# Jason-Hoford/inversus-reinforcement-learning

Measured on NVIDIA B200. Metric: env_steps_per_sec, higher is better.
Workload: dtype u32

## Files before the change

inversus-reinforcement-learning_b200/csrc/inversus_b200.cu:

```cuda
#include "inversus_kernels.cuh"

#include <chrono>
#include <cstdio>
#include <cstdlib>
#include <cstring>
#include <new>
#include <thread>
#include <vector>

using namespace inv;

namespace inv_host {
void expand_f32(const uint32_t *bits, float *dst, int64_t lo, int64_t hi, int nthreads);
int hardware_threads();
bool stage_action_ids(int8_t *dst, const int8_t *src, int64_t n);
bool check_action_ids(const int8_t *src, int64_t n);
}

struct inv_sim {
    inv_config cfg;
    int64_t n;
    uint4 *state;
    void *obs1, *obs2;
    float *extra1, *extra2, *reward;
    uint8_t *done, *info, *dbg;
    int32_t *ep_steps;
    double *ep_return, *reward64;
    uint32_t *status;
    const uint32_t *table;
    int sm_count;
    int64_t launches;
    bool was_reset;
    int8_t *h_a1, *h_a2, *d_a1, *d_a2;
    uint32_t *h_status;
    cudaStream_t host_stream, copy_stream;
    cudaEvent_t ev_last;
    bool ev_last_valid, need_device_sync;
    cudaEvent_t ev_kernel[8], ev_bits[8], ev_t0, ev_t1;
    char *d_small, *h_small;
    size_t small_bytes, off_extra1, off_extra2, off_reward, off_steps, off_return, off_done, off_info;
    int host_threads;
    double dma_frac;
    bool dma_frac_auto;
    uint4 *d_bits[2];
    uint32_t *h_bits[2];
    double last_dma_s, last_expand_s;
    char *d_events;
    int32_t *d_ev_counts;
    int64_t *h_ev_count;
    int64_t ev_guess;
    cudaEvent_t ev_events;
};

static thread_local char g_err[512] = "";

// ... 175 lines not shown
    p.mode = s->cfg.mode;
    p.difficulty = s->cfg.difficulty;
    p.max_steps = s->cfg.max_episode_steps;
    p.auto_reset = (s->cfg.flags & INV_FLAG_AUTO_RESET) ? 1 : 0;
    return p;
}

constexpr int kTileEnvs = 32;
#ifndef INV_BF16_E
#define INV_BF16_E 64
#endif
#ifndef INV_BF16_T
#define INV_BF16_T 128
#endif
#ifndef INV_NARROW_E
#define INV_NARROW_E 128
#endif
#ifndef INV_NARROW_T
#define INV_NARROW_T 128
#endif
#ifndef INV_WIDE_MIN_ENVS
#define INV_WIDE_MIN_ENVS 131072
#endif

template <int OP, int DT, bool P2V, bool INDEXED, int E, int T = kThreads>
cudaError_t launch_one(const Params &p, int sm_count, cudaStream_t st)
{
    (void)sm_count;
    auto kern = inv_kernel<OP, DT, P2V, INDEXED, E, T>;
    constexpr size_t smem = smem_bytes<E, P2V, INDEXED, DT>();
    static bool configured[64] = {};
    int dev = 0;
    cudaGetDevice(&dev);
    if (dev < 0 || dev >= 64 || !configured[dev]) {
        cudaError_t e = cudaFuncSetAttribute(kern, cudaFuncAttributeMaxDynamicSharedMemorySize, (int)smem);
        if (e != cudaSuccess) return e;
        if (dev >= 0 && dev < 64) configured[dev] = true;
    }
    const int64_t ntiles = (p.count + E - 1) / E;
    if (ntiles <= 0) return cudaSuccess;
    const unsigned grid = (unsigned)(ntiles < (int64_t)0x7FFFFFFF ? ntiles : (int64_t)0x7FFFFFFF);
    kern<<<grid, T, smem, st>>>(p);
    return cudaGetLastError();
}

template <int OP, int DT, bool P2V, bool INDEXED>
cudaError_t launch_e(const Params &p, int sm_count, cudaStream_t st)
{
    if constexpr (DT == INV_OBS_NONE && !INDEXED && OP != OP_DEBUG) {
        return launch_one<OP, DT, P2V, false, 128, 128>(p, sm_count, st);
    } else if constexpr (OP == OP_STEP && !INDEXED && DT != INV_OBS_F32) {
        constexpr int E = (DT == INV_OBS_BF16 && !P2V) ? INV_BF16_E : INV_NARROW_E;
        constexpr int T = (DT == INV_OBS_BF16 && !P2V) ? INV_BF16_T : INV_NARROW_T;
        return launch_one<OP_STEP, DT, P2V, false, E, T>(p, sm_count, st);
    } else if constexpr (DT == INV_OBS_F32 && !INDEXED && OP != OP_DEBUG) {
        if (p.count >= INV_WIDE_MIN_ENVS) {
            if constexpr (OP == OP_STEP && !P2V) return launch_one<OP, DT, P2V, false, 64, 256>(p, sm_count, st);
            else if constexpr (OP == OP_STEP) return launch_one<OP, DT, P2V, false, 64, 384>(p, sm_count, st);
            else return launch_one<OP, DT, P2V, false, 128, 512>(p, sm_count, st);
        }
        return launch_one<OP, DT, P2V, INDEXED, kTileEnvs>(p, sm_count, st);
    } else {
        return launch_one<OP, DT, P2V, INDEXED, kTileEnvs>(p, sm_count, st);
    }
}

template <int OP, bool INDEXED>
cudaError_t launch(const Params &p, int dt, bool p2v, int sm_count, cudaStream_t st)
{
#define INV_CASE(DTV)                                                                   \
    case DTV:                                                                           \
        return p2v ? launch_e<OP, DTV, true, INDEXED>(p, sm_count, st)                  \
                   : launch_e<OP, DTV, false, INDEXED>(p, sm_count, st);
// ... 90 lines not shown
        return fail(INV_ERR_INVALID_ARG, "Unknown opponent_type");
    if (cfg->difficulty != INV_DIFFICULTY_EASY && cfg->difficulty != INV_DIFFICULTY_HARD)
        return fail(INV_ERR_INVALID_ARG, "inv_create: difficulty must be easy(0) or hard(1)");
    if (cfg->obs_dtype < INV_OBS_F32 || cfg->obs_dtype > INV_OBS_NONE)
        return fail(INV_ERR_INVALID_ARG, "inv_create: unknown obs_dtype");
    if (cfg->max_episode_steps <= 0) return fail(INV_ERR_INVALID_ARG, "inv_create: max_episode_steps must be positive");
    if (cfg->env_id_base < 0 || cfg->env_id_base + cfg->n_envs > 0xFFFFFFFFll)
        return fail(INV_ERR_INVALID_ARG, "inv_create: global env ids must fit 32 bits");
    int ndev = inv_device_count();
    if (ndev <= 0) return fail(INV_ERR_NO_DEVICE, "no CUDA device: this simulator has no CPU fallback");
    if (cfg->device < 0 || cfg->device >= ndev) return fail(INV_ERR_INVALID_ARG, "inv_create: bad device ordinal");
    DeviceGuard g(cfg->device);
    cudaDeviceProp prop;
    CUDA_TRY(cudaGetDeviceProperties(&prop, cfg->device));
    if (prop.major != 10)
        return fail(INV_ERR_NO_DEVICE, "device is not sm_100 (B200): kernels are built for sm_100a only");

    inv_sim *s = new (std::nothrow) inv_sim();
    if (!s) return fail(INV_ERR_INVALID_ARG, "out of host memory");
    memset(s, 0, sizeof(*s));
    s->cfg = *cfg;
    if (cfg->mode == INV_MODE_SELFPLAY) s->cfg.flags |= INV_FLAG_P2_VIEW;
    s->n = cfg->n_envs;
    s->sm_count = prop.multiProcessorCount;
    s->host_threads = inv_host::hardware_threads() > 32 ? 32 : inv_host::hardware_threads();
    s->dma_frac = 0.35;
    s->dma_frac_auto = true;
    const int64_t n = s->n;
    const bool p2v = (s->cfg.flags & INV_FLAG_P2_VIEW) != 0;
    const size_t obs_bytes = (size_t)n * INV_OBS_ELEMS * obs_elem_bytes(cfg->obs_dtype);
#define ALLOC(ptr, bytes)                                                        \
    do {                                                                         \
        cudaError_t e_ = cudaMalloc((void **)&(ptr), (bytes));                   \
        if (e_ != cudaSuccess) {                                                 \
            fail(INV_ERR_CUDA, "cudaMalloc(%s): %s", #ptr, cudaGetErrorString(e_)); \
            inv_destroy(s);                                                      \
            return INV_ERR_CUDA;                                                 \
        }                                                                        \
    } while (0)
    ALLOC(s->state, (size_t)n * INV_PACKED_STATE_BYTES);
    if (obs_bytes) {
        ALLOC(s->obs1, obs_bytes);
        if (p2v) ALLOC(s->obs2, obs_bytes);
    }
    {
        auto up = [](size_t v) { return (v + 255) & ~(size_t)255; };
// ... 83 lines not shown
}

int inv_get_config(const inv_sim *s, inv_config *out)
{
    if (!s || !out) return fail(INV_ERR_INVALID_ARG, "inv_get_config: null argument");
    *out = s->cfg;
    return INV_OK;
}

static void note_launch(inv_sim *s, cudaStream_t st)
{
    s->launches += 1;
    if (st == s->host_stream) return;
    cudaStreamCaptureStatus cap = cudaStreamCaptureStatusNone;
    if (cudaStreamIsCapturing(st, &cap) != cudaSuccess || cap != cudaStreamCaptureStatusNone ||
        cudaEventRecord(s->ev_last, st) != cudaSuccess) {
        cudaGetLastError();
        s->need_device_sync = true;
        return;
    }
    s->ev_last_valid = true;
}

static int order_host_stream(inv_sim *s)
{
    if (s->need_device_sync) CUDA_TRY(cudaDeviceSynchronize());
    else if (s->ev_last_valid) CUDA_TRY(cudaStreamWaitEvent(s->host_stream, s->ev_last, 0));
    return INV_OK;
}

static Params chunk_params(const Params &b, int64_t first, int64_t count, size_t env_bytes)
{
    Params p = b;
    p.state = b.state + first;
    p.count = count;
    if (b.a1) p.a1 = b.a1 + first;
    if (b.a2) p.a2 = b.a2 + first;
    if (b.table) p.table = b.table + first * INV_TABLE_STRIDE;
    p.obs1 = static_cast<char *>(b.obs1) + (size_t)first * env_bytes;
    if (b.obs2) p.obs2 = static_cast<char *>(b.obs2) + (size_t)first * env_bytes;
    if (b.bits1) p.bits1 = b.bits1 + first * 16;
    if (b.bits2) p.bits2 = b.bits2 + first * 16;
    p.extra1 = b.extra1 + first * 4;
    if (b.extra2) p.extra2 = b.extra2 + first * 4;
    p.reward = b.reward + first;
    if (b.reward64) p.reward64 = b.reward64 + first;
    p.done = b.done + first;
    p.info = b.info + first;
    p.dbg = b.dbg + first;
    p.ep_steps = b.ep_steps + first;
    p.ep_return = b.ep_return + first;
    p.env_id_base = b.env_id_base + (uint32_t)first;
    return p;
}

int inv_reset(inv_sim *s, void *stream)
{
    if (!s) return fail(INV_ERR_INVALID_ARG, "inv_reset: null handle");
    DeviceGuard g(s->cfg.device);
    Params p = base_params(s);
    CUDA_TRY((launch<OP_RESET, false>(p, s->cfg.obs_dtype, (s->cfg.flags & INV_FLAG_P2_VIEW) != 0, s->sm_count,
                                      (cudaStream_t)stream)));
    note_launch(s, (cudaStream_t)stream);
    s->was_reset = true;
    return INV_OK;
}

int inv_reset_envs(inv_sim *s, const int64_t *idx_dev, int64_t count, void *stream)
{
    if (!s || (!idx_dev && count > 0)) return fail(INV_ERR_INVALID_ARG, "inv_reset_envs: null argument");
    if (count < 0 || count > s->n) return fail(INV_ERR_INVALID_ARG, "inv_reset_envs: bad count");
    if (count == 0) return INV_OK;
    DeviceGuard g(s->cfg.device);
    Params p = base_params(s);
    p.idx = idx_dev;
    p.count = count;
    CUDA_TRY((launch<OP_RESET, true>(p, s->cfg.obs_dtype, (s->cfg.flags & INV_FLAG_P2_VIEW) != 0, s->sm_count,
                                     (cudaStream_t)stream)));
    note_launch(s, (cudaStream_t)stream);
    return INV_OK;
}

static int step_impl(inv_sim *s, const int8_t *a1, const int8_t *a2, void *stream, uint4 *bits1, uint4 *bits2,
                     int64_t first, int64_t count)
{
    if (!s || !a1) return fail(INV_ERR_INVALID_ARG, "inv_step: null argument");
    if (!s->was_reset) return fail(INV_ERR_NOT_RESET, "inv_step before inv_reset");
    if (s->cfg.mode == INV_MODE_SELFPLAY && !a2)
        return fail(INV_ERR_INVALID_ARG, "opponent_policy required for selfplay mode");
    DeviceGuard g(s->cfg.device);
    Params p = base_params(s);
    p.a1 = a1;
    p.a2 = a2;
    p.bits1 = bits1;
    p.bits2 = bits2;
    if (first != 0 || count != s->n) p = chunk_params(p, first, count, obs_env_bytes(s->cfg.obs_dtype));
    CUDA_TRY((launch<OP_STEP, false>(p, s->cfg.obs_dtype, (s->cfg.flags & INV_FLAG_P2_VIEW) != 0, s->sm_count,
                                     (cudaStream_t)stream)));
    note_launch(s, (cudaStream_t)stream);
    return INV_OK;
}

int inv_step(inv_sim *s, const int8_t *a1, const int8_t *a2, void *stream)
{
    return step_impl(s, a1, a2, stream, nullptr, nullptr, 0, s ? s->n : 0);
}

constexpr int kMaxHostChunks = 8;
constexpr int64_t kHostChunkMinEnvs = 131072;
constexpr size_t kStagedSmallMax = 8u << 20;

struct SmallOut {
    float *extra_p1, *extra_p2, *reward;
    uint8_t *done, *info;
    int32_t *episode_steps;
    double *episode_return;
};

static int ensure_host_staging(inv_sim *s)
{
    const size_t n = (size_t)s->n;
    if (!s->h_a1) CUDA_TRY(cudaMallocHost((void **)&s->h_a1, n));
    if (!s->h_a2) CUDA_TRY(cudaMallocHost((void **)&s->h_a2, n));
    size_t staged_max = kStagedSmallMax;
    if (const char *e = getenv("INV_HOST_STAGED_MAX")) staged_max = (size_t)atoll(e);
    if (!s->h_small && s->small_bytes <= staged_max) CUDA_TRY(cudaMallocHost((void **)&s->h_small, s->small_bytes));
    return INV_OK;
}
// ... 99 lines not shown
                  double *episode_return)
{
    if (!s) return fail(INV_ERR_INVALID_ARG, "inv_step_host: null argument");
    if (obs_p1 && !s->obs1) return fail(INV_ERR_INVALID_ARG, "this handle keeps no observation tensor (INV_OBS_NONE)");
    if (obs_p2 && !s->obs2) return fail(INV_ERR_INVALID_ARG, "P2 view was not enabled (INV_FLAG_P2_VIEW)");
    if (extra_p2 && !s->extra2) return fail(INV_ERR_INVALID_ARG, "P2 view was not enabled (INV_FLAG_P2_VIEW)");
    DeviceGuard g(s->cfg.device);
    int rc = begin_host_step(s, a1, a2, "inv_step_host");
    if (rc != INV_OK) return rc;
    const int64_t n = s->n;
    const bool selfplay = s->cfg.mode == INV_MODE_SELFPLAY;
    const bool expand = use_host_expand(s, obs_p1, obs_p2);
    if (expand && (rc = ensure_bits_staging(s, obs_p2 != nullptr)) != INV_OK) return rc;
    cudaStream_t ks = s->host_stream, cs = s->copy_stream;
    int64_t bounds[kMaxHostChunks + 1];
    const int nchunks = host_chunk_bounds(n, obs_p1 || obs_p2, s->h_small != nullptr, bounds);
    const SmallOut so = {extra_p1, extra_p2, reward, done, info, episode_steps, episode_return};
    const size_t env_bytes = (size_t)INV_OBS_ELEMS * obs_elem_bytes(s->cfg.obs_dtype);
    void *dst[2] = {obs_p1, obs_p2};
    const void *src[2] = {s->obs1, s->obs2};
    const double frac = expand ? s->dma_frac : 1.0;
    int64_t lo[kMaxHostChunks], mid[kMaxHostChunks], hi[kMaxHostChunks];

    int used = 0;
    for (int c = 0; c < nchunks; ++c) {
        const int64_t first = bounds[c];
        if (first >= n) break;
        const int64_t count = bounds[c + 1] - first;
        if (count <= 0) break;
        lo[c] = first;
        hi[c] = first + count;
        mid[c] = expand ? first + ((int64_t)((double)count * frac) & ~(int64_t)255) : first + count;
        rc = step_impl(s, s->d_a1, selfplay ? s->d_a2 : nullptr, ks, expand ? s->d_bits[0] : nullptr,
                       expand && obs_p2 ? s->d_bits[1] : nullptr, first, count);
        if (rc != INV_OK) return rc;
        CUDA_TRY(cudaEventRecord(s->ev_kernel[c], ks));
        used = c + 1;
    }
    CUDA_TRY(cudaEventRecord(s->ev_t0, cs));
    for (int c = 0; c < used; ++c) {
        CUDA_TRY(cudaStreamWaitEvent(cs, s->ev_kernel[c], 0));
        if ((rc = copy_small_outputs(s, cs, so, lo[c], hi[c] - lo[c])) != INV_OK) return rc;
        if (expand) {
            for (int v = 0; v < 2; ++v)
                if (dst[v] && hi[c] > mid[c])
                    CUDA_TRY(cudaMemcpyAsync(s->h_bits[v] + (size_t)mid[c] * 64, s->d_bits[v] + (size_t)mid[c] * 16,
                                             (size_t)(hi[c] - mid[c]) * 256, cudaMemcpyDeviceToHost, cs));
            CUDA_TRY(cudaEventRecord(s->ev_bits[c], cs));
        }
        for (int v = 0; v < 2; ++v)
            if (dst[v] && mid[c] > lo[c])
                CUDA_TRY(cudaMemcpyAsync(static_cast<char *>(dst[v]) + (size_t)lo[c] * env_bytes,
                                         static_cast<const char *>(src[v]) + (size_t)lo[c] * env_bytes,
                                         (size_t)(mid[c] - lo[c]) * env_bytes, cudaMemcpyDeviceToHost, cs));
    }
    CUDA_TRY(cudaEventRecord(s->ev_t1, cs));

    double expand_s = 0.0;
    if (expand) {
        using clk = std::chrono::steady_clock;
        for (int c = 0; c < used; ++c) {
// ... 40 lines not shown

int inv_step_host_events(inv_sim *s, const int8_t *a1, const int8_t *a2, float *reward, uint8_t *done,
                         uint8_t *info, inv_episode_event *events, int64_t capacity, int64_t *n_events)
{
    if (!s || !events || !n_events || capacity < 0)
        return fail(INV_ERR_INVALID_ARG, "inv_step_host_events: null handle, events or n_events, or negative capacity");
    DeviceGuard g(s->cfg.device);
    static const bool trace = getenv("INV_HOST_TRACE") != nullptr;
    const auto t_in = std::chrono::steady_clock::now();
    auto lap = [&](const char *what) {
        if (trace)
            fprintf(stderr, "[inv_step_host_events] %-22s %8.1f us\n", what,
                    std::chrono::duration<double, std::micro>(std::chrono::steady_clock::now() - t_in).count());
    };
    int rc = begin_host_step(s, a1, a2, "inv_step_host_events");
    if (rc != INV_OK) return rc;
    lap("ids checked + staged");
    if ((rc = ensure_event_buffers(s)) != INV_OK) return rc;
    const int64_t n = s->n;
    const bool selfplay = s->cfg.mode == INV_MODE_SELFPLAY;
    cudaStream_t ks = s->host_stream, cs = s->copy_stream;
    int64_t bounds[kMaxHostChunks + 1];
    const int nchunks = host_chunk_bounds(n, false, false, bounds);
    int used = 0;
    for (int c = 0; c < nchunks; ++c) {
        const int64_t first = bounds[c], count = bounds[c + 1] - first;
        if (first >= n || count <= 0) break;
        if ((rc = step_impl(s, s->d_a1, selfplay ? s->d_a2 : nullptr, ks, nullptr, nullptr, first, count)) != INV_OK) return rc;
        CUDA_TRY(cudaEventRecord(s->ev_kernel[c], ks));
        used = c + 1;
    }
    {
        const unsigned nblocks = (unsigned)((n + kEvBlockEnvs - 1) / kEvBlockEnvs);
        int64_t *header = reinterpret_cast<int64_t *>(s->d_events);
        inv_episode_event *recs = reinterpret_cast<inv_episode_event *>(s->d_events + kEvHeaderBytes);
        episode_count_kernel<<<nblocks, kEvThreads, 0, ks>>>(s->done, n, s->d_ev_counts);
        episode_write_kernel<<<nblocks, kEvThreads, 0, ks>>>(s->done, s->info, s->ep_steps, s->ep_return, n,
                                                             s->d_ev_counts, header, recs);
        CUDA_TRY(cudaGetLastError());
        s->launches += 2;
        CUDA_TRY(cudaEventRecord(s->ev_events, ks));
    }
    for (int c = 0; c < used; ++c) {
        const size_t f = (size_t)bounds[c], cnt = (size_t)(bounds[c + 1] - bounds[c]);
        CUDA_TRY(cudaStreamWaitEvent(cs, s->ev_kernel[c], 0));
        if (reward) CUDA_TRY(cudaMemcpyAsync(reward + f, s->reward + f, cnt * 4, cudaMemcpyDeviceToHost, cs));
        if (done) CUDA_TRY(cudaMemcpyAsync(done + f, s->done + f, cnt, cudaMemcpyDeviceToHost, cs));
        if (info) CUDA_TRY(cudaMemcpyAsync(info + f, s->info + f, cnt, cudaMemcpyDeviceToHost, cs));
    }
    const char *recs = s->d_events + kEvHeaderBytes;
    const int64_t guess = s->ev_guess < capacity ? s->ev_guess : capacity;
    CUDA_TRY(cudaStreamWaitEvent(cs, s->ev_events, 0));
    CUDA_TRY(cudaMemcpyAsync(s->h_ev_count, s->d_events, sizeof(int64_t), cudaMemcpyDeviceToHost, cs));
    if (guess > 0)
// ... 127 lines not shown
                            (size_t)count * 16, cudaMemcpyDeviceToHost));
        pl[k] = dst;
    }
    for (int64_t i = 0; i < count; ++i) unpack_host(pl, i, &out[i]);
    return INV_OK;
}

int inv_import_state(inv_sim *s, const inv_env_state *in, int64_t first, int64_t count)
{
    if (!s || !in) return fail(INV_ERR_INVALID_ARG, "inv_import_state: null argument");
    if (first < 0 || count < 0 || first + count > s->n) return fail(INV_ERR_INVALID_ARG, "inv_import_state: bad range");
    if (count == 0) return INV_OK;
    DeviceGuard g(s->cfg.device);
    std::vector<uint32_t> buf((size_t)count * 20);
    uint32_t *pl[5];
    for (int k = 0; k < 5; ++k) pl[k] = buf.data() + (size_t)k * count * 4;
    for (int64_t i = 0; i < count; ++i)
        if (!pack_host(&in[i], pl, i)) return fail(INV_ERR_INVALID_ARG, "inv_import_state: field out of range");
    CUDA_TRY(cudaDeviceSynchronize());
    for (int k = 0; k < 5; ++k)
        CUDA_TRY(cudaMemcpy(reinterpret_cast<char *>(s->state) + ((size_t)k * s->n + first) * 16, pl[k],
                            (size_t)count * 16, cudaMemcpyHostToDevice));
    s->was_reset = true;
    return INV_OK;
}

int inv_load_packed_state(inv_sim *s, const void *packed_dev, void *stream)
{
    if (!s || !packed_dev) return fail(INV_ERR_INVALID_ARG, "inv_load_packed_state: null argument");
    DeviceGuard g(s->cfg.device);
    CUDA_TRY(cudaMemcpyAsync(s->state, packed_dev, (size_t)s->n * INV_PACKED_STATE_BYTES, cudaMemcpyDeviceToDevice,
                             (cudaStream_t)stream));
    s->was_reset = true;
    return INV_OK;
}

int inv_obs_from_packed(inv_sim *s, const void *packed_dev, int64_t stride, int64_t count, int view, int obs_dtype,
                        void *obs_out, float *extra_out, void *stream)
{
    if (!s || !packed_dev || !obs_out || !extra_out) return fail(INV_ERR_INVALID_ARG, "inv_obs_from_packed: null argument");
    if (count < 0 || stride < count || (view != 0 && view != 1)) return fail(INV_ERR_INVALID_ARG, "inv_obs_from_packed: bad argument");
    if (count == 0) return INV_OK;
    DeviceGuard g(s->cfg.device);
    Params p = base_params(s);
    p.state_in = static_cast<const uint4 *>(packed_dev);
    p.stride = stride;
    p.count = count;
    p.view = view;
    p.obs1 = obs_out;
    p.extra1 = extra_out;
    p.table = nullptr;
    cudaError_t ce;
    switch (obs_dtype) {
    case INV_OBS_F32: ce = launch_e<OP_OBS, INV_OBS_F32, false, false>(p, s->sm_count, (cudaStream_t)stream); break;
    case INV_OBS_BF16: ce = launch_e<OP_OBS, INV_OBS_BF16, false, false>(p, s->sm_count, (cudaStream_t)stream); break;
    case INV_OBS_U8: ce = launch_e<OP_OBS, INV_OBS_U8, false, false>(p, s->sm_count, (cudaStream_t)stream); break;
    default: return fail(INV_ERR_INVALID_ARG, "inv_obs_from_packed: unknown obs_dtype");
    }
    CUDA_TRY(ce);
    note_launch(s, (cudaStream_t)stream);
    return INV_OK;
}

int inv_debug_phase(inv_sim *s, int phase, int pid, int arg, int arg2, void *stream)
{
    if (!s) return fail(INV_ERR_INVALID_ARG, "inv_debug_phase: null handle");
    if (phase < 0 || phase > INV_PHASE_DUMMY_POLICY || (pid != 0 && pid != 1))
        return fail(INV_ERR_INVALID_ARG, "inv_debug_phase: bad phase or pid");
    if ((phase <= INV_PHASE_WIDE_SHOT) && (arg < 0 || arg > 3)) return fail(INV_ERR_INVALID_ARG, "inv_debug_phase: bad direction");
    if (phase == INV_PHASE_STEP_PLAYERS && (arg < 0 || arg > 12 || arg2 < 0 || arg2 > 12))
        return fail(INV_ERR_INVALID_ACTION, "Invalid action_id: must be 0-12");
    DeviceGuard g(s->cfg.device);
    Params p = base_params(s);
    p.phase = phase; p.pid = pid; p.arg = arg; p.arg2 = arg2;
    CUDA_TRY((launch_one<OP_DEBUG, INV_OBS_F32, false, false, 32>(p, s->sm_count, (cudaStream_t)stream)));
    note_launch(s, (cudaStream_t)stream);
    return INV_OK;
}

int inv_poll_status(inv_sim *s, void *stream, uint32_t *bits)
{
    if (!s || !bits) return fail(INV_ERR_INVALID_ARG, "inv_poll_status: null argument");
    DeviceGuard g(s->cfg.device);
    cudaStream_t st = (cudaStream_t)stream;
    CUDA_TRY(cudaMemcpyAsync(s->h_status, s->status, 4, cudaMemcpyDeviceToHost, st));
    CUDA_TRY(cudaMemsetAsync(s->status, 0, 4, st));
    CUDA_TRY(cudaStreamSynchronize(st));
    *bits = *s->h_status;
    return INV_OK;
}

int64_t inv_launch_count(const inv_sim *s) { return s ? s->launches : 0; }

int inv_gae(const float *reward_dev, const float *value_dev, const uint8_t *done_dev, const float *last_value_dev,
            double gamma, double lam, int32_t T, int64_t N, float *adv_dev, float *ret_dev, void *stream)
{
    if (!reward_dev || !value_dev || !done_dev || !adv_dev || !ret_dev || T < 0 || N < 0)
        return fail(INV_ERR_INVALID_ARG, "inv_gae: bad argument");
    if (T == 0 || N == 0) return INV_OK;
// ... 9 lines not shown
```

inversus-reinforcement-learning_b200/csrc/inversus_kernels.cuh:

```cuda
#pragma once

#ifdef INV_HOST_BUILD
#include "host_shim.h"
#else
#include <cuda_runtime.h>
#endif
#include <stdint.h>

#include "../../include/inversus_b200.h"

namespace inv {

constexpr int kW = INV_BOARD_W;
constexpr int kH = INV_BOARD_H;
constexpr int kTiles = kW * kH;
constexpr int kMaxAmmo = 6;
constexpr int kReloadTicks = 30;
constexpr int kWideCost = 3;
constexpr int kSlots = INV_MAX_BULLETS;
constexpr int kRowWords = 57;
constexpr int kThreads = 128;

constexpr uint32_t kThreshShootHard = 858993460u;
constexpr uint32_t kThreshRandMoveHard = 214748365u;
constexpr uint32_t kThreshMoveEasy = 4294968u;

enum : int { OP_STEP = 0, OP_RESET = 1, OP_OBS = 2, OP_DEBUG = 3 };

__constant__ double kProximity[24] = {
    0x1.0624dd2f1a9fcp-9,  0x1.f75104d551d69p-10, 0x1.e2584f4c6e6dap-10, 0x1.cd5f99c38b04bp-10,
    0x1.b866e43aa79bcp-10, 0x1.a36e2eb1c432dp-10, 0x1.8e757928e0c9ep-10, 0x1.797cc39ffd60ep-10,
    0x1.64840e1719f7fp-10, 0x1.4f8b588e368f1p-10, 0x1.3a92a30553261p-10, 0x1.2599ed7c6fbd3p-10,
    0x1.10a137f38c544p-10, 0x1.f75104d551d69p-11, 0x1.cd5f99c38b04ap-11, 0x1.a36e2eb1c432dp-11,
    0x1.797cc39ffd60ep-11, 0x1.4f8b588e368f0p-11, 0x1.2599ed7c6fbd3p-11, 0x1.f75104d551d69p-12,
    0x1.a36e2eb1c432bp-12, 0x1.4f8b588e368f2p-12, 0x1.f75104d551d69p-13, 0x1.4f8b588e368eep-13};
__constant__ float kAmmoNorm[8] = {0x0.0p+0f, 0x1.555556p-3f, 0x1.555556p-2f, 0x1.0p-1f,
                                   0x1.555556p-1f, 0x1.aaaaaap-1f, 0x1.0p+0f, 0x1.2aaaaap+0f};

struct Params {
    uint4 *state;
    const uint4 *state_in;
    int64_t stride;
    int64_t count;
    const int64_t *idx;
    const int8_t *a1, *a2;
    const uint32_t *table;
    void *obs1, *obs2;
    uint4 *bits1, *bits2;
    float *extra1, *extra2;
    float *reward;
// ... 337 lines not shown
    if (c1 >= 0) {
        if (dr.below(2) == 0) { const int t = c0; c0 = c1; c1 = t; }
    }
    if (c0 >= 0 && p2_can_step(s, c0)) return 1 + c0;
    if (c1 >= 0 && p2_can_step(s, c1)) return 1 + c1;
    dirs = shuffle4(dirs, dr);
#pragma unroll
    for (int i = 0; i < 4; ++i) {
        const int c = (dirs >> (2 * i)) & 3u;
        if (p2_can_step(s, c)) return 1 + c;
    }
    return 0;
}

__device__ __forceinline__ float ammo_norm(int k) { return kAmmoNorm[k & 7]; }
__device__ __forceinline__ float4 extra_vec(const Env &s, int viewer)
{
    const int e = 1 - viewer;
    return make_float4(s.alive[viewer] ? ammo_norm(s.ammo[viewer]) : 0.0f,
                       s.alive[e] ? ammo_norm(s.ammo[e]) : 0.0f,
                       s.alive[viewer] ? 1.0f : 0.0f, s.alive[e] ? 1.0f : 0.0f);
}

template <int E>
__device__ __forceinline__ void build_row(uint32_t *row, const Env &s, const uint16_t *sb, int viewer)
{
    const uint32_t *t = s.t;
    row[0] = ~t[0]; row[1] = ~t[1]; row[2] = ~t[2]; row[3] = ~t[3];
    row[4] = (~t[4] & 0x3FFFFFu) | (t[0] << 22);
    row[5] = (t[0] >> 10) | (t[1] << 22);
    row[6] = (t[1] >> 10) | (t[2] << 22);
    row[7] = (t[2] >> 10) | (t[3] << 22);
    row[8] = (t[3] >> 10) | (t[4] << 22);
    row[9] = (t[4] >> 10);
#pragma unroll
    for (int k = 10; k < kRowWords; ++k) row[k] = 0u;
    const int e = 1 - viewer;
    if (s.alive[viewer]) { const int b = 2 * kTiles + s.y[viewer] * kW + s.x[viewer]; row[b >> 5] |= 1u << (b & 31); }
    if (s.alive[e])      { const int b = 3 * kTiles + s.y[e] * kW + s.x[e];           row[b >> 5] |= 1u << (b & 31); }
    for (int i = 0; i < s.nb; ++i) {
        const uint32_t bl = sb[i * E];
        const int ch = ((((bl >> 10) & 1u) == (uint32_t)viewer) ? 4 : 8) + (int)((bl >> 8) & 3u);
        const int b = ch * kTiles + (int)((bl >> 4) & 15u) * kW + (int)(bl & 15u);
        row[b >> 5] |= 1u << (b & 31);
    }
}


struct StepResult {
    float reward;
    double reward64;
    uint8_t done, info;
    int32_t ep_steps;
    double ep_return;
};

__device__ __forceinline__ void rl_reset(Env &s, const Params &p, uint32_t gid, const uint32_t *trow)
{
    s.episode += 1u;
    Draws dr;
    dr.init(p, gid, s.episode, INV_STREAM_RESET, trow ? trow + INV_TABLE_RESET_OFF : nullptr);
    engine_reset(s, dr);
    s.step = 0u;
    s.ret = 0.0;
}

template <int E>
// ... 112 lines not shown

#ifndef INV_ST_PLAIN
#define INV_ST_PLAIN 0
#endif
#if INV_ST_PLAIN
__device__ __forceinline__ void st_stream(uint4 *p, uint4 v) { *p = v; }
__device__ __forceinline__ void st_stream(uint2 *p, uint2 v) { *p = v; }
#else
__device__ __forceinline__ void st_stream(uint4 *p, uint4 v) { __stcs(p, v); }
__device__ __forceinline__ void st_stream(uint2 *p, uint2 v) { __stcs(p, v); }
#endif
template <> struct ObsFmt<INV_OBS_NONE> {
    static constexpr int kChunks = 1, kBits = 0;
    typedef uint4 chunk_t;
    static __device__ __forceinline__ chunk_t expand(uint32_t) { return make_uint4(0u, 0u, 0u, 0u); }
};
__device__ __forceinline__ void st_stream(uint8v *p, uint8v v)
{
    asm volatile("st.global.v8.b32 [%0], {%1,%2,%3,%4,%5,%6,%7,%8};" ::"l"(p), "r"(v.lo.x), "r"(v.lo.y), "r"(v.lo.z),
                 "r"(v.lo.w), "r"(v.hi.x), "r"(v.hi.y), "r"(v.hi.z), "r"(v.hi.w)
                 : "memory");
}

template <int E, bool P2V, bool INDEXED, int DT = INV_OBS_F32>
constexpr size_t smem_bytes()
{
    return (DT == INV_OBS_NONE ? 0 : (size_t)E * kRowWords * 4 * (P2V ? 2 : 1)) + (size_t)kSlots * E * 2 +
           (INDEXED ? (size_t)E * 8 : 0);
}

template <int OP, int DT, bool P2V, bool INDEXED, int E, int T = kThreads>
__global__ void __launch_bounds__(T) inv_kernel(const Params p)
{
    static_assert(E <= T && E % 32 == 0 && T % 32 == 0, "tile must be whole warps");
    extern __shared__ __align__(16) uint32_t smem[];
    constexpr bool kObs = DT != INV_OBS_NONE;
    uint32_t *rows1 = smem;
    uint32_t *rows2 = rows1 + (P2V && kObs ? E * kRowWords : 0);
    uint16_t *sbul = reinterpret_cast<uint16_t *>(rows2 + (kObs ? E * kRowWords : 0));
    int64_t *s_env = reinterpret_cast<int64_t *>(sbul + kSlots * E);
    typedef ObsFmt<DT> Fmt;
    typedef typename Fmt::chunk_t chunk_t;

    const int tid = threadIdx.x;
    const int64_t ntiles = (p.count + E - 1) / E;

    for (int64_t tile = blockIdx.x; tile < ntiles; tile += gridDim.x) {
        const int64_t base = tile * E;
        const int nvalid = (int)min((int64_t)E, p.count - base);

        bool live = tid < nvalid;
        if (INDEXED && live) {
            const int64_t cand = p.idx[base + tid];
            if ((uint64_t)cand >= (uint64_t)p.stride) {
                atomicOr(p.status, INV_STATUS_BAD_INDEX);
                s_env[tid] = -1;
                live = false;
            }
        }
        if (live) {
            const int64_t ei = INDEXED ? p.idx[base + tid] : base + tid;
            if (INDEXED) s_env[tid] = ei;
            uint16_t *sb = sbul + tid;
            uint32_t *row1 = rows1 + tid * kRowWords;
            Env s;
            load_env<E>(s, sb, OP == OP_OBS ? p.state_in : p.state, p.stride, ei);
            const uint32_t gid = p.env_id_base + (uint32_t)ei;
            const uint32_t *trow = p.table ? p.table + ei * INV_TABLE_STRIDE : nullptr;

            if (OP == OP_STEP) {
                const StepResult o = rl_step<E>(s, sb, p.a1[ei], p.mode == INV_MODE_DUMMY ? 0 : p.a2[ei], p, gid, trow);
                p.reward[ei] = o.reward;
                if (p.reward64) p.reward64[ei] = o.reward64;
                p.done[ei] = o.done;
                p.info[ei] = o.info;
                p.ep_steps[ei] = o.ep_steps;
                p.ep_return[ei] = o.ep_return;
            } else if (OP == OP_RESET) {
                rl_reset(s, p, gid, trow);
            } else if (OP == OP_DEBUG) {
                int res = 0;
                switch (p.phase) {
                case INV_PHASE_TRY_MOVE:
                    res = p.pid ? try_move(s, 1, p.arg) : try_move(s, 0, p.arg);
                    break;
                case INV_PHASE_SPAWN_BULLET:
                    res = p.pid ? spawn_bullet<E>(s, sb, 1, p.arg, p.status) : spawn_bullet<E>(s, sb, 0, p.arg, p.status);
                    break;
                case INV_PHASE_WIDE_SHOT:
                    res = p.pid ? spawn_wide_shot<E>(s, sb, 1, p.arg, p.status) : spawn_wide_shot<E>(s, sb, 0, p.arg, p.status);
                    break;
                case INV_PHASE_RELOAD: reload_ammo(s); break;
                case INV_PHASE_UPDATE_BULLETS: update_bullets<E>(s, sb); break;
// ... 3 lines not shown
                    Draws dr;
                    dr.init(p, gid, s.episode, INV_STREAM_RESET, trow ? trow + INV_TABLE_RESET_OFF : nullptr);
                    engine_reset(s, dr);
                    break;
                }
                case INV_PHASE_DUMMY_POLICY: {
                    Draws dr;
                    dr.init(p, gid, s.episode, s.step, trow);
                    res = dummy_policy(s, dr, p.difficulty);
                    break;
                }
                default: break;
                }
                p.dbg[ei] = (uint8_t)res;
            }

            if (OP != OP_OBS) store_env<E>(s, sb, p.state, p.stride, ei);

            if (OP != OP_DEBUG) {
                const int64_t eo = (OP == OP_OBS) ? base + tid : ei;
                if (OP == OP_OBS && p.view) {
                    if (kObs) build_row<E>(row1, s, sb, 1);
                    reinterpret_cast<float4 *>(p.extra1)[eo] = extra_vec(s, 1);
                } else {
                    if (kObs) build_row<E>(row1, s, sb, 0);
                    reinterpret_cast<float4 *>(p.extra1)[eo] = extra_vec(s, 0);
                }
                if (P2V) {
                    if (kObs) build_row<E>(rows2 + tid * kRowWords, s, sb, 1);
                    reinterpret_cast<float4 *>(p.extra2)[eo] = extra_vec(s, 1);
                }
            }
        }
        if (OP == OP_DEBUG || !kObs) continue;
        __syncthreads();

#pragma unroll 1
        for (int v = 0; v < (P2V ? 2 : 1); ++v) {
            const uint32_t *rows = v ? rows2 : rows1;
            chunk_t *out = reinterpret_cast<chunk_t *>(v ? p.obs2 : p.obs1);
            const int total = nvalid * Fmt::kChunks;
            if (!INDEXED) {
                chunk_t *o = out + base * Fmt::kChunks;
#pragma unroll 4
                for (int g = tid; g < total; g += T) {
                    const int e = g / Fmt::kChunks;
                    const int bit = (g - e * Fmt::kChunks) * Fmt::kBits;
                    const uint32_t w = rows[e * kRowWords + (bit >> 5)] >> (bit & 31);
                    st_stream(o + g, Fmt::expand(w));
                }
            } else {
#pragma unroll 2
                for (int g = tid; g < total; g += T) {
                    const int e = g / Fmt::kChunks;
                    const int c = g - e * Fmt::kChunks;
                    const int bit = c * Fmt::kBits;
                    if (s_env[e] < 0) continue;
// ... 33 lines not shown
```

Before: 935.0 million.

## Write only changed observation chunks in step via pre/post XOR delta

Adds an OP_STEP_DELTA kernel that builds each env's observation bit row before the step, XORs it with the row after the step, and stores only the output chunks whose bits changed. The previous observation buffer is assumed to still be valid. Host-side staleness tracking (reset, state load, debug calls, obs written into own buffers, graph capture) falls back to the full write when that assumption may not hold. This aims to cut DRAM write traffic for the large observation tensor, at the cost of extra row building and compare work per env and the correctness risk of missed staleness cases.

Measured after the change: 2.506 billion, median of 6. 2.68x the previous value.

```diff
diff --git a/inversus-reinforcement-learning_b200/csrc/inversus_b200.cu b/inversus-reinforcement-learning_b200/csrc/inversus_b200.cu
--- a/inversus-reinforcement-learning_b200/csrc/inversus_b200.cu
+++ b/inversus-reinforcement-learning_b200/csrc/inversus_b200.cu
@@ -31,6 +31,7 @@
     int sm_count;
     int64_t launches;
     bool was_reset;
+    bool obs_stale, obs_stale_captured;
     int8_t *h_a1, *h_a2, *d_a1, *d_a2;
     uint32_t *h_status;
     cudaStream_t host_stream, copy_stream;
@@ -252,6 +253,12 @@
 #ifndef INV_WIDE_MIN_ENVS
 #define INV_WIDE_MIN_ENVS 131072
 #endif
+#ifndef INV_DELTA_E
+#define INV_DELTA_E 128
+#endif
+#ifndef INV_DELTA_MIN_ENVS
+#define INV_DELTA_MIN_ENVS 65536
+#endif
 
 template <int OP, int DT, bool P2V, bool INDEXED, int E, int T = kThreads>
 cudaError_t launch_one(const Params &p, int sm_count, cudaStream_t st)
@@ -277,8 +284,12 @@
 template <int OP, int DT, bool P2V, bool INDEXED>
 cudaError_t launch_e(const Params &p, int sm_count, cudaStream_t st)
 {
-    if constexpr (DT == INV_OBS_NONE && !INDEXED && OP != OP_DEBUG) {
+    if constexpr (OP == OP_STEP_DELTA && DT == INV_OBS_NONE) {
+        return launch_e<OP_STEP, DT, P2V, INDEXED>(p, sm_count, st);
+    } else if constexpr (DT == INV_OBS_NONE && !INDEXED && OP != OP_DEBUG) {
         return launch_one<OP, DT, P2V, false, 128, 128>(p, sm_count, st);
+    } else if constexpr (OP == OP_STEP_DELTA) {
+        return launch_one<OP, DT, P2V, false, INV_DELTA_E, INV_DELTA_E>(p, sm_count, st);
     } else if constexpr (OP == OP_STEP && !INDEXED && DT != INV_OBS_F32) {
         constexpr int E = (DT == INV_OBS_BF16 && !P2V) ? INV_BF16_E : INV_NARROW_E;
         constexpr int T = (DT == INV_OBS_BF16 && !P2V) ? INV_BF16_T : INV_NARROW_T;
@@ -415,6 +426,7 @@
     s->cfg = *cfg;
     if (cfg->mode == INV_MODE_SELFPLAY) s->cfg.flags |= INV_FLAG_P2_VIEW;
     s->n = cfg->n_envs;
+    s->obs_stale = true;
     s->sm_count = prop.multiProcessorCount;
     s->host_threads = inv_host::hardware_threads() > 32 ? 32 : inv_host::hardware_threads();
     s->dma_frac = 0.35;
@@ -544,6 +556,28 @@
     s->ev_last_valid = true;
 }
 
+static bool stream_capturing(cudaStream_t st)
+{
+    cudaStreamCaptureStatus cap = cudaStreamCaptureStatusNone;
+    if (cudaStreamIsCapturing(st, &cap) != cudaSuccess) {
+        cudaGetLastError();
+        return true;
+    }
+    return cap != cudaStreamCaptureStatusNone;
+}
+
+static void mark_obs_stale(inv_sim *s, cudaStream_t st)
+{
+    s->obs_stale = true;
+    if (stream_capturing(st)) s->obs_stale_captured = true;
+}
+
+static bool step_writes_full_obs(const inv_sim *s, bool captured)
+{
+    return s->obs_stale || s->obs_stale_captured || captured || s->cfg.obs_dtype == INV_OBS_U8 ||
+           s->n < INV_DELTA_MIN_ENVS;
+}
+
 static int order_host_stream(inv_sim *s)
 {
     if (s->need_device_sync) CUDA_TRY(cudaDeviceSynchronize());
@@ -581,10 +615,12 @@
     if (!s) return fail(INV_ERR_INVALID_ARG, "inv_reset: null handle");
     DeviceGuard g(s->cfg.device);
     Params p = base_params(s);
+    const bool captured = stream_capturing((cudaStream_t)stream);
     CUDA_TRY((launch<OP_RESET, false>(p, s->cfg.obs_dtype, (s->cfg.flags & INV_FLAG_P2_VIEW) != 0, s->sm_count,
                                       (cudaStream_t)stream)));
     note_launch(s, (cudaStream_t)stream);
     s->was_reset = true;
+    if (!captured) s->obs_stale = false;
     return INV_OK;
 }
 
@@ -604,7 +640,7 @@
 }
 
 static int step_impl(inv_sim *s, const int8_t *a1, const int8_t *a2, void *stream, uint4 *bits1, uint4 *bits2,
-                     int64_t first, int64_t count)
+                     int64_t first, int64_t count, bool full_obs)
 {
     if (!s || !a1) return fail(INV_ERR_INVALID_ARG, "inv_step: null argument");
     if (!s->was_reset) return fail(INV_ERR_NOT_RESET, "inv_step before inv_reset");
@@ -617,15 +653,22 @@
     p.bits1 = bits1;
     p.bits2 = bits2;
     if (first != 0 || count != s->n) p = chunk_params(p, first, count, obs_env_bytes(s->cfg.obs_dtype));
-    CUDA_TRY((launch<OP_STEP, false>(p, s->cfg.obs_dtype, (s->cfg.flags & INV_FLAG_P2_VIEW) != 0, s->sm_count,
-                                     (cudaStream_t)stream)));
+    const bool p2v = (s->cfg.flags & INV_FLAG_P2_VIEW) != 0;
+    if (full_obs || bits1 || bits2)
+        CUDA_TRY((launch<OP_STEP, false>(p, s->cfg.obs_dtype, p2v, s->sm_count, (cudaStream_t)stream)));
+    else
+        CUDA_TRY((launch<OP_STEP_DELTA, false>(p, s->cfg.obs_dtype, p2v, s->sm_count, (cudaStream_t)stream)));
     note_launch(s, (cudaStream_t)stream);
     return INV_OK;
 }
 
 int inv_step(inv_sim *s, const int8_t *a1, const int8_t *a2, void *stream)
 {
-    return step_impl(s, a1, a2, stream, nullptr, nullptr, 0, s ? s->n : 0);
+    if (!s) return fail(INV_ERR_INVALID_ARG, "inv_step: null argument");
+    const bool captured = stream_capturing((cudaStream_t)stream);
+    const int rc = step_impl(s, a1, a2, stream, nullptr, nullptr, 0, s->n, step_writes_full_obs(s, captured));
+    if (rc == INV_OK && !captured) s->obs_stale = false;
+    return rc;
 }
 
 constexpr int kMaxHostChunks = 8;
@@ -771,6 +814,7 @@
     const double frac = expand ? s->dma_frac : 1.0;
     int64_t lo[kMaxHostChunks], mid[kMaxHostChunks], hi[kMaxHostChunks];
 
+    const bool full_obs = step_writes_full_obs(s, false) || expand;
     int used = 0;
     for (int c = 0; c < nchunks; ++c) {
         const int64_t first = bounds[c];
@@ -781,11 +825,12 @@
         hi[c] = first + count;
         mid[c] = expand ? first + ((int64_t)((double)count * frac) & ~(int64_t)255) : first + count;
         rc = step_impl(s, s->d_a1, selfplay ? s->d_a2 : nullptr, ks, expand ? s->d_bits[0] : nullptr,
-                       expand && obs_p2 ? s->d_bits[1] : nullptr, first, count);
+                       expand && obs_p2 ? s->d_bits[1] : nullptr, first, count, full_obs);
         if (rc != INV_OK) return rc;
         CUDA_TRY(cudaEventRecord(s->ev_kernel[c], ks));
         used = c + 1;
     }
+    s->obs_stale = false;
     CUDA_TRY(cudaEventRecord(s->ev_t0, cs));
     for (int c = 0; c < used; ++c) {
         CUDA_TRY(cudaStreamWaitEvent(cs, s->ev_kernel[c], 0));
@@ -872,14 +917,17 @@
     cudaStream_t ks = s->host_stream, cs = s->copy_stream;
     int64_t bounds[kMaxHostChunks + 1];
     const int nchunks = host_chunk_bounds(n, false, false, bounds);
+    const bool full_obs = step_writes_full_obs(s, false);
     int used = 0;
     for (int c = 0; c < nchunks; ++c) {
         const int64_t first = bounds[c], count = bounds[c + 1] - first;
         if (first >= n || count <= 0) break;
-        if ((rc = step_impl(s, s->d_a1, selfplay ? s->d_a2 : nullptr, ks, nullptr, nullptr, first, count)) != INV_OK) return rc;
+        if ((rc = step_impl(s, s->d_a1, selfplay ? s->d_a2 : nullptr, ks, nullptr, nullptr, first, count, full_obs)) != INV_OK)
+            return rc;
         CUDA_TRY(cudaEventRecord(s->ev_kernel[c], ks));
         used = c + 1;
     }
+    s->obs_stale = false;
     {
         const unsigned nblocks = (unsigned)((n + kEvBlockEnvs - 1) / kEvBlockEnvs);
         int64_t *header = reinterpret_cast<int64_t *>(s->d_events);
@@ -1053,6 +1101,7 @@
         CUDA_TRY(cudaMemcpy(reinterpret_cast<char *>(s->state) + ((size_t)k * s->n + first) * 16, pl[k],
                             (size_t)count * 16, cudaMemcpyHostToDevice));
     s->was_reset = true;
+    s->obs_stale = true;
     return INV_OK;
 }
 
@@ -1063,6 +1112,7 @@
     CUDA_TRY(cudaMemcpyAsync(s->state, packed_dev, (size_t)s->n * INV_PACKED_STATE_BYTES, cudaMemcpyDeviceToDevice,
                              (cudaStream_t)stream));
     s->was_reset = true;
+    mark_obs_stale(s, (cudaStream_t)stream);
     return INV_OK;
 }
 
@@ -1090,6 +1140,12 @@
     }
     CUDA_TRY(ce);
     note_launch(s, (cudaStream_t)stream);
+    const char *o = static_cast<const char *>(obs_out), *o_end = o + (size_t)count * obs_env_bytes(obs_dtype);
+    const size_t own = (size_t)s->n * obs_env_bytes(s->cfg.obs_dtype);
+    for (const void *b : {s->obs1, s->obs2}) {
+        const char *lo = static_cast<const char *>(b);
+        if (lo && o < lo + own && lo < o_end) mark_obs_stale(s, (cudaStream_t)stream);
+    }
     return INV_OK;
 }
 
@@ -1106,6 +1162,7 @@
     p.phase = phase; p.pid = pid; p.arg = arg; p.arg2 = arg2;
     CUDA_TRY((launch_one<OP_DEBUG, INV_OBS_F32, false, false, 32>(p, s->sm_count, (cudaStream_t)stream)));
     note_launch(s, (cudaStream_t)stream);
+    mark_obs_stale(s, (cudaStream_t)stream);
     return INV_OK;
 }
 
diff --git a/inversus-reinforcement-learning_b200/csrc/inversus_kernels.cuh b/inversus-reinforcement-learning_b200/csrc/inversus_kernels.cuh
--- a/inversus-reinforcement-learning_b200/csrc/inversus_kernels.cuh
+++ b/inversus-reinforcement-learning_b200/csrc/inversus_kernels.cuh
@@ -25,7 +25,7 @@
 constexpr uint32_t kThreshRandMoveHard = 214748365u;
 constexpr uint32_t kThreshMoveEasy = 4294968u;
 
-enum : int { OP_STEP = 0, OP_RESET = 1, OP_OBS = 2, OP_DEBUG = 3 };
+enum : int { OP_STEP = 0, OP_RESET = 1, OP_OBS = 2, OP_DEBUG = 3, OP_STEP_DELTA = 4 };
 
 __constant__ double kProximity[24] = {
     0x1.0624dd2f1a9fcp-9,  0x1.f75104d551d69p-10, 0x1.e2584f4c6e6dap-10, 0x1.cd5f99c38b04bp-10,
@@ -409,27 +409,70 @@
                        s.alive[viewer] ? 1.0f : 0.0f, s.alive[e] ? 1.0f : 0.0f);
 }
 
-template <int E>
-__device__ __forceinline__ void build_row(uint32_t *row, const Env &s, const uint16_t *sb, int viewer)
-{
-    const uint32_t *t = s.t;
-    row[0] = ~t[0]; row[1] = ~t[1]; row[2] = ~t[2]; row[3] = ~t[3];
-    row[4] = (~t[4] & 0x3FFFFFu) | (t[0] << 22);
-    row[5] = (t[0] >> 10) | (t[1] << 22);
-    row[6] = (t[1] >> 10) | (t[2] << 22);
-    row[7] = (t[2] >> 10) | (t[3] << 22);
-    row[8] = (t[3] >> 10) | (t[4] << 22);
-    row[9] = (t[4] >> 10);
-#pragma unroll
-    for (int k = 10; k < kRowWords; ++k) row[k] = 0u;
+constexpr int kTileRowWords = 10;
+__device__ __forceinline__ uint32_t tile_row_word(const uint32_t *t, int k)
+{
+    switch (k) {
+    case 0: case 1: case 2: case 3: return ~t[k];
+    case 4: return (~t[4] & 0x3FFFFFu) | (t[0] << 22);
+    case 5: case 6: case 7: case 8: return (t[k - 5] >> 10) | (t[k - 4] << 22);
+    case 9: return t[4] >> 10;
+    default: return 0u;
+    }
+}
+
+template <int E, class F>
+__device__ __forceinline__ void for_each_sparse_bit(const Env &s, const uint16_t *sb, int viewer, F &&f)
+{
     const int e = 1 - viewer;
-    if (s.alive[viewer]) { const int b = 2 * kTiles + s.y[viewer] * kW + s.x[viewer]; row[b >> 5] |= 1u << (b & 31); }
-    if (s.alive[e])      { const int b = 3 * kTiles + s.y[e] * kW + s.x[e];           row[b >> 5] |= 1u << (b & 31); }
+    if (s.alive[viewer]) f(2 * kTiles + s.y[viewer] * kW + s.x[viewer]);
+    if (s.alive[e]) f(3 * kTiles + s.y[e] * kW + s.x[e]);
     for (int i = 0; i < s.nb; ++i) {
         const uint32_t bl = sb[i * E];
         const int ch = ((((bl >> 10) & 1u) == (uint32_t)viewer) ? 4 : 8) + (int)((bl >> 8) & 3u);
-        const int b = ch * kTiles + (int)((bl >> 4) & 15u) * kW + (int)(bl & 15u);
-        row[b >> 5] |= 1u << (b & 31);
+        f(ch * kTiles + (int)((bl >> 4) & 15u) * kW + (int)(bl & 15u));
+    }
+}
+
+template <int E>
+__device__ __forceinline__ void build_row(uint32_t *row, const Env &s, const uint16_t *sb, int viewer)
+{
+#pragma unroll
+    for (int k = 0; k < kTileRowWords; ++k) row[k] = tile_row_word(s.t, k);
+#pragma unroll
+    for (int k = kTileRowWords; k < kRowWords; ++k) row[k] = 0u;
+    for_each_sparse_bit<E>(s, sb, viewer, [&](int b) { row[b >> 5] |= 1u << (b & 31); });
+}
+
+template <int E>
+__device__ __forceinline__ void xor_row(uint32_t *d, const Env &s, const uint16_t *sb, int viewer)
+{
+#pragma unroll
+    for (int k = 0; k < kTileRowWords; ++k) d[k] ^= tile_row_word(s.t, k);
+    for_each_sparse_bit<E>(s, sb, viewer, [&](int b) { d[b >> 5] ^= 1u << (b & 31); });
+}
+
+template <int E>
+__device__ __forceinline__ uint32_t sparse_row_word(const Env &s, const uint16_t *sb, int viewer, int k)
+{
+    uint32_t w = 0u;
+    for_each_sparse_bit<E>(s, sb, viewer, [&](int b) { w |= (b >> 5) == k ? 1u << (b & 31) : 0u; });
+    return w;
+}
+
+template <int E, class F>
+__device__ __forceinline__ void for_each_changed_word(const uint32_t *d, const Env &s, const uint16_t *sb, int viewer,
+                                                      F &&put)
+{
+#pragma unroll
+    for (int k = 0; k < kTileRowWords; ++k) {
+        const uint32_t x = d[k];
+        if (x) put(k, x, tile_row_word(s.t, k) | (k == kTileRowWords - 1 ? sparse_row_word<E>(s, sb, viewer, k) : 0u));
+    }
+#pragma unroll 1
+    for (int k = kTileRowWords; k < kRowWords; ++k) {
+        const uint32_t x = d[k];
+        if (x) put(k, x, sparse_row_word<E>(s, sb, viewer, k));
     }
 }
 
@@ -588,6 +631,20 @@
                  : "memory");
 }
 
+template <int DT, int E>
+__device__ __forceinline__ void store_changed_chunks(const uint32_t *d, const Env &s, const uint16_t *sb, int viewer,
+                                                     typename ObsFmt<DT>::chunk_t *out)
+{
+    typedef ObsFmt<DT> Fmt;
+    constexpr int kPerWord = 32 / Fmt::kBits;
+    constexpr uint32_t kMask = (1u << Fmt::kBits) - 1u;
+    for_each_changed_word<E>(d, s, sb, viewer, [&](int k, uint32_t x, uint32_t w) {
+#pragma unroll
+        for (int j = 0; j < kPerWord; ++j)
+            if ((x >> (j * Fmt::kBits)) & kMask) st_stream(out + k * kPerWord + j, Fmt::expand(w >> (j * Fmt::kBits)));
+    });
+}
+
 template <int E, bool P2V, bool INDEXED, int DT = INV_OBS_F32>
 constexpr size_t smem_bytes()
 {
@@ -601,6 +658,9 @@
     static_assert(E <= T && E % 32 == 0 && T % 32 == 0, "tile must be whole warps");
     extern __shared__ __align__(16) uint32_t smem[];
     constexpr bool kObs = DT != INV_OBS_NONE;
+    constexpr bool kStep = OP == OP_STEP || OP == OP_STEP_DELTA;
+    constexpr bool kDelta = OP == OP_STEP_DELTA;
+    static_assert(!kDelta || (E == T && kObs && !INDEXED), "the delta step is thread-per-env with an observation");
     uint32_t *rows1 = smem;
     uint32_t *rows2 = rows1 + (P2V && kObs ? E * kRowWords : 0);
     uint16_t *sbul = reinterpret_cast<uint16_t *>(rows2 + (kObs ? E * kRowWords : 0));
@@ -633,8 +693,13 @@
             load_env<E>(s, sb, OP == OP_OBS ? p.state_in : p.state, p.stride, ei);
             const uint32_t gid = p.env_id_base + (uint32_t)ei;
             const uint32_t *trow = p.table ? p.table + ei * INV_TABLE_STRIDE : nullptr;
-
-            if (OP == OP_STEP) {
+            uint32_t *row2 = rows2 + tid * kRowWords;
+
+            if constexpr (kDelta) {
+                build_row<E>(row1, s, sb, 0);
+                if (P2V) build_row<E>(row2, s, sb, 1);
+            }
+            if (kStep) {
                 const StepResult o = rl_step<E>(s, sb, p.a1[ei], p.mode == INV_MODE_DUMMY ? 0 : p.a2[ei], p, gid, trow);
                 p.reward[ei] = o.reward;
                 if (p.reward64) p.reward64[ei] = o.reward64;
@@ -684,17 +749,26 @@
                 if (OP == OP_OBS && p.view) {
                     if (kObs) build_row<E>(row1, s, sb, 1);
                     reinterpret_cast<float4 *>(p.extra1)[eo] = extra_vec(s, 1);
+                } else if constexpr (kDelta) {
+                    xor_row<E>(row1, s, sb, 0);
+                    store_changed_chunks<DT, E>(row1, s, sb, 0, reinterpret_cast<chunk_t *>(p.obs1) + ei * Fmt::kChunks);
+                    reinterpret_cast<float4 *>(p.extra1)[eo] = extra_vec(s, 0);
                 } else {
                     if (kObs) build_row<E>(row1, s, sb, 0);
                     reinterpret_cast<float4 *>(p.extra1)[eo] = extra_vec(s, 0);
                 }
                 if (P2V) {
-                    if (kObs) build_row<E>(rows2 + tid * kRowWords, s, sb, 1);
+                    if constexpr (kDelta) {
+                        xor_row<E>(row2, s, sb, 1);
+                        store_changed_chunks<DT, E>(row2, s, sb, 1, reinterpret_cast<chunk_t *>(p.obs2) + ei * Fmt::kChunks);
+                    } else if (kObs) {
+                        build_row<E>(row2, s, sb, 1);
+                    }
                     reinterpret_cast<float4 *>(p.extra2)[eo] = extra_vec(s, 1);
                 }
             }
         }
-        if (OP == OP_DEBUG || !kObs) continue;
+        if (OP == OP_DEBUG || !kObs || kDelta) continue;
         __syncthreads();
 
 #pragma unroll 1
diff --git a/profiles/measure_obs_delta.py b/profiles/measure_obs_delta.py
--- /dev/null
+++ b/profiles/measure_obs_delta.py
@@ -0,0 +1,148 @@
+import argparse
+import json
+import os
+import subprocess
+import sys
+
+ROOT = os.path.dirname(os.path.dirname(os.path.abspath(__file__)))
+sys.path.insert(0, ROOT)
+
+N_ACTION_SETS = 16
+SECTOR = 32
+
+
+def gpu_info():
+    q = "name,power.limit,clocks.max.sm"
+    try:
+        out = subprocess.run(["nvidia-smi", f"--query-gpu={q}", "--format=csv,noheader", "-i", "0"],
+                             capture_output=True, text=True, timeout=60).stdout.strip()
+        name, power, clock = [x.strip() for x in out.split(",")]
+        return {"name": name, "power_limit": power, "sm_max_clock": clock}
+    except Exception as e:
+        return {"name": None, "error": repr(e)}
+
+
+def memset_gbs(torch):
+    fill = torch.empty(1 << 30, dtype=torch.float32, device="cuda")
+    for _ in range(2):
+        fill.zero_()
+    e0, e1 = torch.cuda.Event(enable_timing=True), torch.cuda.Event(enable_timing=True)
+    e0.record()
+    for _ in range(5):
+        fill.zero_()
+    e1.record()
+    torch.cuda.synchronize()
+    gbs = 5 * fill.numel() * 4 / (e0.elapsed_time(e1) * 1e-3) / 1e9
+    del fill
+    torch.cuda.empty_cache()
+    return gbs
+
+
+def changed_units(before, after, elems):
+    a, b = before.reshape(-1), after.reshape(-1)
+    pad = (-a.numel()) % elems
+    ne = a != b
+    if pad:
+        ne = torch_pad(ne, pad)
+    return int(ne.view(-1, elems).any(dim=1).sum().item())
+
+
+def torch_pad(t, pad):
+    import torch
+    return torch.cat([t, torch.zeros(pad, dtype=t.dtype, device=t.device)])
+
+
+def measure(torch, BatchedInversus, mode, dtype, n, timed, count_steps, seed):
+    selfplay = mode == "selfplay"
+    sim = BatchedInversus(n, mode, "hard", 500, seed=seed, device=0, obs_dtype=dtype, auto_reset=True)
+    g = torch.Generator(device="cuda")
+    g.manual_seed(seed * 1000)
+    acts = [torch.randint(0, 13, (n,), device="cuda", dtype=torch.int8, generator=g) for _ in range(N_ACTION_SETS)]
+    acts2 = [torch.randint(0, 13, (n,), device="cuda", dtype=torch.int8, generator=g)
+             for _ in range(N_ACTION_SETS)] if selfplay else None
+    t = 0
+
+    def step():
+        nonlocal t
+        k = t % N_ACTION_SETS
+        sim.step(acts[k], acts2[k] if selfplay else None)
+        t += 1
+
+    sim.reset()
+    for _ in range(600):
+        step()
+    torch.cuda.synchronize()
+    views = [sim.obs] + ([sim.obs_p2] if selfplay else [])
+    esize = views[0].element_size()
+    chunks = lines = 0
+    for _ in range(count_steps):
+        before = [v.clone() for v in views]
+        step()
+        for b, v in zip(before, views):
+            chunks += changed_units(b, v, 8)
+            lines += changed_units(b, v, 128 // esize)
+        del before
+    torch.cuda.empty_cache()
+    for _ in range(20):
+        step()
+    ev = [torch.cuda.Event(enable_timing=True) for _ in range(2)]
+    torch.cuda.synchronize()
+    ev[0].record()
+    for _ in range(timed):
+        step()
+    ev[1].record()
+    torch.cuda.synchronize()
+    ms = ev[0].elapsed_time(ev[1]) / timed
+    assert sim.poll_status() == 0
+    sim.close()
+    nv = len(views)
+    r = {"config": f"{mode}_{dtype}", "envs": n, "kernel_ms": ms, "timed_launches": timed,
+         "env_steps_per_s": n / (ms * 1e-3)}
+    if count_steps:
+        c = chunks / (n * count_steps)
+        small = 160 + (2 if selfplay else 1) + 4 + 1 + 1 + 4 + 8 + 16 * nv
+        model = small + SECTOR * c
+        r.update({"count_steps": count_steps, "views": nv,
+                  "changed_chunks_per_env_step": c, "chunks_per_env_step": 225 * nv,
+                  "changed_128B_lines_per_env_step": lines / (n * count_steps),
+                  "lines_per_env_step": 1800 * esize / 128 * nv,
+                  "modelled_dram_bytes_per_env_step": model,
+                  "full_write_obs_bytes_per_env_step": 1800 * esize * nv,
+                  "modelled_gbs": model * n / (ms * 1e-3) / 1e9})
+    return r
+
+
+def main():
+    ap = argparse.ArgumentParser()
+    ap.add_argument("--envs", type=int, default=1 << 20)
+    ap.add_argument("--configs", default="dummy_f32,selfplay_f32,dummy_bf16,dummy_u8")
+    ap.add_argument("--timed", type=int, default=200)
+    ap.add_argument("--count-steps", type=int, default=20)
+    ap.add_argument("--seed", type=int, default=0)
+    ap.add_argument("--out", default=None, help="also append the JSON lines to this file")
+    args = ap.parse_args()
+    import torch
+    if not torch.cuda.is_available() or torch.cuda.device_count() < 1:
+        sys.exit("measure_obs_delta.py: no CUDA device")
+    from inversus_b200 import BatchedInversus, _capi
+    gpu = gpu_info()
+    gpu["torch_name"] = torch.cuda.get_device_name(0)
+    lines = [{"gpu": gpu, "library": _capi.library_path()}]
+    for cfg in args.configs.split(","):
+        mode, dtype = cfg.split("_")
+        lines.append(measure(torch, BatchedInversus, mode, dtype, args.envs, args.timed, args.count_steps, args.seed))
+        print(json.dumps(lines[-1]), flush=True)
+    ceil = memset_gbs(torch)
+    lines[0]["memset_gbs"] = ceil
+    for r in lines[1:]:
+        if "modelled_gbs" in r:
+            r["modelled_frac_of_memset"] = r["modelled_gbs"] / ceil
+    print(json.dumps(lines[0]), flush=True)
+    if args.out:
+        with open(args.out, "a") as f:
+            for r in lines:
+                f.write(json.dumps(r) + "\n")
+
+
+if __name__ == "__main__":
+    main()
```
